# grunwaldlab/krisp

Measured on AMD Instinct MI355X. Metric: k-mers/s sorted+intersected at k=28, higher is better.
Workload: dtype u64

## Files before the change

### include/krisp_hip.h

```cpp
#ifndef KRISP_HIP_H
#define KRISP_HIP_H

#include <stddef.h>
#include <stdint.h>

#ifdef __cplusplus
extern "C" {
#endif

typedef struct kr_ctx kr_ctx;

typedef struct { uint64_t prefix, in_mask, out_mask; } kr_cand;

typedef struct { uint64_t key; uint32_t genome; uint32_t count; } kr_record;

enum {
    KR_OK = 0,
    KR_ERR_HIP = -1,
    KR_ERR_PARAM = -2,
    KR_ERR_CAPACITY = -3,
    KR_ERR_STATE = -4,
    KR_ERR_KEY = -5,
    KR_ERR_HOST = -6
};
// ... 193 lines not shown
       KR_OPT_COARSE_POOL = 12,
       KR_OPT_JOIN2 = 13,
       KR_OPT_WIDE_ORDERED = 6 };
int     kr_set_option(kr_ctx*, int option, int64_t value);

int     kr_sync(kr_ctx*);
int     kr_timer_begin(kr_ctx*);
double  kr_timer_end_ms(kr_ctx*);
int     kr_stage_enable(kr_ctx*, int on);
int     kr_stage_select(kr_ctx*, unsigned stage_mask);
int     kr_stage_reset(kr_ctx*);
double  kr_stage_ms(kr_ctx*, int stage);
int64_t kr_stage_launches(kr_ctx*, int stage);

int64_t kr_debug_fetch(kr_ctx*, int genome_id, int what, void* out, size_t cap_bytes);
int64_t kr_debug_inversions(kr_ctx*, int genome_id);
double  kr_debug_localsort(kr_ctx*, int genome_id, int reps, int mode);
double  kr_debug_intersect(kr_ctx*, const int* genome_ids, int n, const uint8_t* is_ingroup, int reps, int mode);
double  kr_debug_copy_gbps(kr_ctx*, size_t bytes, int reps);
const char* kr_debug_copy_which(kr_ctx*);
int     kr_build_experiments(void);
int     kr_debug_lazy(kr_ctx*, int64_t* out8);
int     kr_debug_isect(kr_ctx*, int64_t* out8);
int     kr_debug_scan(kr_ctx*, int64_t* out8);
int     kr_debug_place(kr_ctx*, double* out8);
int     kr_debug_coarse_pool(kr_ctx*, double* out8);
int     kr_debug_comm(kr_ctx*, int64_t* out8);
int     kr_debug_comm_probe(kr_ctx*, size_t bytes, int reps, double* out3);
int64_t kr_debug_cands_selfexchange(kr_ctx*, int apply_filter);
int     kr_debug_comm_hang(kr_ctx*);
int64_t kr_debug_budget_left(kr_ctx*);
int     kr_debug_budget_set(kr_ctx*, int64_t left);
int     kr_debug_info(kr_ctx*, int64_t* out8);

#ifdef __cplusplus
}
#endif
#endif
```

### krisp_amd/_native.py

```python
import ctypes
import os

import numpy as np

HERE = os.path.dirname(os.path.abspath(__file__))
LIB_PATH = os.environ.get("KRISP_HIP_LIB") or os.path.join(HERE, "libkrisp_hip.so")

CAND = np.dtype([("prefix", "<u8"), ("in_mask", "<u8"), ("out_mask", "<u8")])
RECORD = np.dtype([("key", "<u8"), ("genome", "<u4"), ("count", "<u4")])
WIDE_HIT = np.dtype([("cand", "<u4"), ("genome", "<u4"), ("pos", "<u4"), ("strand", "<u4")])
LOC_HIT = np.dtype([("group", "<u4"), ("strand", "<u4"), ("pos", "<u8")])
NEAR_HIT = np.dtype([("target", "<u4"), ("strand", "u1"), ("mismatches", "u1"), ("flank_mismatches", "u1"), ("pad", "u1"),
                     ("pos", "<u8")])
PRODUCT_SITE = np.dtype([("pos", "<u8"), ("entry", "<u4"), ("mismatches", "u1"), ("end_mismatches", "u1"),
                         ("pad", "<u2")])
PRODUCT_HIT = np.dtype([("pos", "<u8"), ("length", "<u4"), ("pair", "<u4"), ("strand", "u1"), ("left_mm", "u1"),
                        ("right_mm", "u1"), ("left_end_mm", "u1"), ("right_end_mm", "u1"), ("pad", "u1", (3,))])
DESIGN_RECORD = np.dtype([("found", "<u4"), ("product_size", "<u4"), ("pair_penalty", "<u4"), ("left_start", "<u2"),
                          ("left_len", "<u2"), ("right_start", "<u2"), ("right_len", "<u2"), ("left_tm", "<i4"), ("right_tm", "<i4"),
                          ("left_gc", "<u2"), ("right_gc", "<u2"), ("left_penalty", "<u4"), ("right_penalty", "<u4"),
                          ("left_self_any", "<i4"), ("left_self_end", "<i4"), ("right_self_any", "<i4"),
                          ("right_self_end", "<i4"), ("pair_any", "<i4"), ("pair_end", "<i4")])
DESIGN_RECORD_HP = np.dtype(DESIGN_RECORD.descr + [("left_hairpin", "<i4"), ("right_hairpin", "<i4")])
GUIDE_RECORD = np.dtype([("found", "<u4"), ("strand", "<u4"), ("start", "<u4"), ("min_mismatches", "<u4"),
# ... 125 lines not shown
    ("kr_timer_end_ms", _c.c_double, [_P]),
    ("kr_stage_enable", _c.c_int, [_P, _c.c_int]),
    ("kr_stage_select", _c.c_int, [_P, _c.c_uint]),
    ("kr_stage_reset", _c.c_int, [_P]),
    ("kr_stage_ms", _c.c_double, [_P, _c.c_int]),
    ("kr_stage_launches", _c.c_int64, [_P, _c.c_int]),
    ("kr_debug_fetch", _c.c_int64, [_P, _c.c_int, _c.c_int, _P, _c.c_size_t]),
    ("kr_debug_inversions", _c.c_int64, [_P, _c.c_int]),
    ("kr_debug_localsort", _c.c_double, [_P, _c.c_int, _c.c_int, _c.c_int]),
    ("kr_debug_intersect", _c.c_double, [_P, _P, _c.c_int, _P, _c.c_int, _c.c_int]),
    ("kr_debug_copy_gbps", _c.c_double, [_P, _c.c_size_t, _c.c_int]),
    ("kr_debug_copy_which", _c.c_char_p, [_P]),
    ("kr_mem_info", _c.c_int, [_P, _P]),
    ("kr_debug_comm", _c.c_int, [_P, _P]),
    ("kr_debug_place", _c.c_int, [_P, _P]),
    ("kr_debug_coarse_pool", _c.c_int, [_P, _P]),
    ("kr_debug_comm_probe", _c.c_int, [_P, _c.c_size_t, _c.c_int, _P]),
    ("kr_debug_cands_selfexchange", _c.c_int64, [_P, _c.c_int]),
    ("kr_debug_info", _c.c_int, [_P, _P]),
    ("kr_render_records", _c.c_int64, [_P, _c.c_size_t, _c.c_int, _c.c_int, _c.c_int, _P, _c.c_size_t, _P, _c.c_size_t, _P,
                                       _c.c_int, _P, _P, _P, _P]),
    ("kr_text_free", None, [_P]),
    ("kr_debug_isect", _c.c_int, [_P, _P]),
    ("kr_debug_lazy", _c.c_int, [_P, _P]),
    ("kr_debug_scan", _c.c_int, [_P, _P]),
    ("kr_set_mixed_alphabets", _c.c_int, [_P, _c.c_int]),
    ("kr_build_experiments", _c.c_int, []),
    ("kr_comm_set_timeout", _c.c_int, [_P, _c.c_int]),
    ("kr_debug_comm_hang", _c.c_int, [_P]),
    ("kr_debug_budget_left", _c.c_int64, [_P]),
    ("kr_debug_budget_set", _c.c_int, [_P, _c.c_int64]),
]


class GuideParams(ctypes.Structure):
    _fields_ = [("guide_size", _c.c_int32), ("pam5_len", _c.c_int32), ("pam3_len", _c.c_int32), ("pam5", _c.c_uint8 * 8),
                ("pam3", _c.c_uint8 * 8), ("gc_lo", _c.c_int32), ("gc_hi", _c.c_int32), ("min_mismatches", _c.c_int32)]


class KrispHipError(RuntimeError):
    code = None


ERR_CAPACITY = -3


# ... 629 lines not shown
        for n in names:
            mask |= 1 << STAGES.index(n)
        self.lib.kr_stage_select(self.ctx, mask)

    def stage_reset(self):
        self.lib.kr_stage_reset(self.ctx)

    def stage_times(self):
        return {name: (self.lib.kr_stage_ms(self.ctx, i), self.lib.kr_stage_launches(self.ctx, i))
                for i, name in enumerate(STAGES)}

    def debug_info(self):
        o = np.zeros(8, dtype=np.int64)
        self.lib.kr_debug_info(self.ctx, _ptr(o))
        return dict(b=int(o[0]), nbuckets=int(o[1]), T=int(o[2]), CAP=int(o[3]), nwg=int(o[4]),
                    overflow_segments=int(o[5]), fallback_launches=int(o[6]), nslices=int(o[7]))

    def debug_isect(self):
        o = np.zeros(8, dtype=np.int64)
        self.lib.kr_debug_isect(self.ctx, _ptr(o))
        return dict(chunk_kernel_items=int(o[0]), slices_redone=int(o[1]), threads=int(o[2]), buckets_per_item_log2=int(o[3]),
                    heads32=int(o[4]), sort_lanes=int(o[5]), join2_launches=int(o[6]), join2_handed_on=int(o[7]))

    def debug_lazy(self):
        o = np.zeros(8, dtype=np.int64)
        self.lib.kr_debug_lazy(self.ctx, _ptr(o))
        return dict(skipped=int(o[0]), ordered_later=int(o[1]), touch_collects=int(o[2]), on=int(o[3]),
                    anchor_in_bucket_order=int(o[4]), fuse_anchor=int(o[5]), coarse=int(o[6]), coarse_promoted=int(o[7]))

    def debug_scan(self):
        o = np.zeros(8, dtype=np.int64)
        self.lib.kr_debug_scan(self.ctx, _ptr(o))
        return dict(tiles=int(o[0]), grid=int(o[1]), cap=int(o[2]), blocks=int(o[3]))

    def copy_gbps(self, nbytes=1 << 30, reps=10):
        v = self.lib.kr_debug_copy_gbps(self.ctx, nbytes, reps)
        if v < 0:
            raise KrispHipError("kr_debug_copy_gbps failed")
        return v

    def mem_info(self):
        o = np.zeros(4, dtype=np.int64)
        self._check(self.lib.kr_mem_info(self.ctx, _ptr(o)), "kr_mem_info")
        return dict(avail=int(o[0]), total=int(o[1]), used=int(o[2]), budget=int(o[3]))

    def debug_comm(self):
# ... 44 lines not shown
```

### krisp_amd/csrc/h_core.inc

```
static thread_local std::string g_last_error;

struct DevBuf {
    void* p = nullptr;
    size_t bytes = 0;
};

struct Slice {
    DevBuf keys, off, chunkstart, chunkdesc, ovf;
    u64 nmax = 0;
    u32 nchunks = 0;
    int64_t count = -1;
    int res = -1;
};

struct Genome {
    int id = -1;
    size_t n_bases = 0;
    u64 nwords = 0;
    u64 nmax = 0;
    DevBuf bases, wkeys;
    DevBuf wlcnt;
    bool wlist = false;
    u32 wlcap = 0;
    std::vector<Slice> sl;
// ... 63 lines not shown
    bool stage_on = false;
    unsigned stage_mask = ~0u;
    struct Pair { hipEvent_t a, b; int stage; };
    std::vector<Pair> pending;
    std::vector<hipEvent_t> pool;
    double stage_ms[KR_ST_COUNT] = {0};
    int64_t stage_n[KR_ST_COUNT] = {0};
    int64_t fallback_launches = 0, overflow_segments = 0;
    int dbg = 0;
    int isect_kernel = 0;
    int ncu = 256;
    DevBuf bgz_in, bgz_tab, bgz_stat;
    DevBuf tx_scan;
    DevBuf tx_text, tx_tile, tx_tilepos, tx_lines, tx_ls, tx_ll, tx_op, tx_outpos, tx_state, tx_tsum, tx_tpos;
    u32* mbox = nullptr;
    std::vector<uint64_t> coltab_host;
    std::vector<int> mb_free;
    int mb_next = 0;
    int i3_occ[3][4][9] = {{{0}}};
    DevBuf isovf;
    int join2 = 1;
    u32 j2_grid = 0;
    int j2_occ[9] = {0};
    int64_t j2_launches = 0, j2_full = 0;
    bool j2_full_counted = false;
    int64_t isect_ovf_items = 0, isect_refall = 0;
    int i3_last_T = 0, i3_last_mlog = 0, i3_last_tags = 0, i3_last_ua = 0;
    int64_t isect_ua = 0;
    int fuse_anchor = 1;
    u32 i3_ovf_cap = I3_OVF_CAP;
    int isect_fmt = 0;
    int opt_slice_bases = -1;
    hipEvent_t slice_ready[2] = {nullptr, nullptr};
    bool custom_layout = false;
    bool mixed_alphabets = false;
    int lazy_order = 1;
    bool order_wanted = false;
    int64_t lazy_skipped = 0, lazy_ordered = 0, lazy_touch = 0;
    DevBuf touchdesc, touchovf;
    int coarse_rest = 1;
    int64_t coarse_done = 0, coarse_promoted = 0;
    int coarse_pool = 1;
    struct PoolBuf { DevBuf buf; double ms; hipEvent_t ev; bool wait; };
    std::vector<PoolBuf> cpool_free;
    int cpool_total = 0;
    int64_t cpool_partitions = 0;
// ... 457 lines not shown
    }
    c->stream = c->lanes[0].stream;
    return c;
}

int kr_comm_destroy(kr_ctx* c);

void kr_destroy(kr_ctx* c) {
    if (!c) return;
    (void)kr_comm_destroy(c);
    (void)hipSetDevice(c->device);
    (void)hipDeviceSynchronize();
    resolve_stages(c);
    for (int i = 0; i < MAX_LANES; i++) {
        Lane& ln = c->lanes[i];
        DevBuf* lb[] = {&ln.codes, &ln.bad, &ln.partial8, &ln.base1, &ln.tmpkeys, &ln.tp, &ln.tiledesc, &ln.tilehist, &ln.wkeys,
                        &ln.pass0, &ln.base64, &ln.partial16, &ln.cursor, &ln.h16exc, &ln.slt, &ln.offa, &ln.cura};
        for (DevBuf* b : lb) release(c, *b);
    }
    for (auto& kv : c->genomes) release_genome(c, kv.second);
    coarse_pool_release(c);
    DevBuf* all[] = {&c->candA, &c->candB, &c->chunkcnt,
                     &c->chunkpos, &c->flags, &c->blockcnt, &c->blockpos, &c->other, &c->records, &c->nrec, &c->fbdesc, &c->fbsegs,
                     &c->coltab, &c->collo, &c->colcnt, &c->colpos, &c->coltsum, &c->coltpos, &c->colfirst, &c->colfm, &c->isovf,
                     &c->bgz_in, &c->bgz_tab, &c->bgz_stat, &c->tx_scan, &c->tx_text, &c->tx_tile, &c->tx_tilepos, &c->tx_lines, &c->tx_ls, &c->tx_ll, &c->tx_op, &c->tx_outpos, &c->tx_state,
                     &c->tx_tsum, &c->tx_tpos, &c->candP, &c->touchdesc, &c->touchovf, &c->co_state, &c->co_tab};
    for (DevBuf* b : all) release(c, *b);
    {
        auto& w = c->wide;
        DevBuf* wb[] = {&w.fin.keys, &w.fin.idx, &w.fin.slots, &w.masks, &w.keep, &w.cnt, &w.hitoff, &w.cursor, &w.hits,
                        &w.cibuf, &w.loc, &w.loccur, &w.tsum, &w.tpos, &w.wcount, &w.flbuf, &w.rows, &w.rowtab};
        for (DevBuf* b : wb) release(c, *b);
        for (int f = 0; f < 2; f++)
            for (int q = 0; q < 2 * FR_MAXP - 1; q++) {
                auto& d = w.fd[f][q];
                release(c, d.keys); release(c, d.idx); release(c, d.slots); release(c, d.mzT); release(c, d.mzB);
            }
    }
    {
        kr_ctx::Bufs sb;
        c->loc.bufs(sb); c->near.bufs(sb); c->ghit.bufs(sb); c->gbulge.bufs(sb); c->prod.bufs(sb); c->prim.bufs(sb);
        for (DevBuf* b : sb) release(c, *b);
        auto& ds = c->design;
        DevBuf* db[] = {&ds.par, &ds.tmpl, &ds.rec, &ds.hprec};
        for (DevBuf* b : db) release(c, *b);
        auto& gu = c->guides;
        DevBuf* gb[] = {&gu.rows, &gu.off, &gu.bnd, &gu.rec};
// ... 1274 lines not shown
```

### krisp_amd/csrc/h_intersect.inc

```
static int64_t intersect_once(kr_ctx* c, const int* ids, int n, const uint8_t* is_in, int apply_filter, bool* redo);

static int64_t cands_merge_device(kr_ctx* c, size_t m, int have_other, int apply_filter);

static inline int fmode(const kr_ctx* c, int apply_filter) { return apply_filter ? (c->mixed_alphabets ? 2 : 1) : 0; }

int kr_set_mixed_alphabets(kr_ctx* c, int on) {
    if (!c) return KR_ERR_PARAM;
    c->mixed_alphabets = on != 0;
    return KR_OK;
}

#define KR_MAX_CANDS 0xFFFFFF00ull
static int cands_fit(kr_ctx* c, uint64_t n, const char* who) {
    if (n < KR_MAX_CANDS) return KR_OK;
    return fail(c, KR_ERR_CAPACITY, "%s: a candidate list of %llu entries exceeds the %llu a list may hold (an intersection that "
                "nothing prunes: give both ingroup and outgroup genomes to one call, or fewer genomes per call)", who,
                (unsigned long long)n, (unsigned long long)KR_MAX_CANDS);
}

static int cands_compact_room(kr_ctx* c, u32 n) {
    const size_t nblk = ((size_t)n + 255) / 256;
    int rc;
    if ((rc = ensure(c, c->flags, (size_t)n * 4))) return rc;
    if ((rc = ensure(c, c->blockcnt, (nblk + 2) * 4))) return rc;
// ... 299 lines not shown
            const int mlog = ip.mlog;
            const u32 T = ip.T;
            const bool tagk = ip.tagk;
            const bool ua = tagk && !gs[anchor]->ordered;
            a3.n = n;
            a3.ingroup_bits = ingroup_bits;
            a3.anchor = anchor;
            a3.apply_filter = a.apply_filter;
            for (int i = 0; i < n; i++) { a3.keys[i] = a.keys[i]; a3.off[i] = a.off[i]; }
            a3.nb = nbk;
            a3.mlog = mlog;
            a3.nitems = (nbk + (1u << mlog) - 1) >> mlog;
            a3.sh = tagk ? ip.sht : std::max(g.rb + mlog - (int)I3_NB_LOG, ip.p0);
            a3.p0 = ip.p0;
            a3.tmp = (kr_cand*)c->candA.p;
            a3.itemcnt = (u32*)c->chunkcnt.p;
            a3.ovf = (u32*)c->isovf.p;
            a3.ovf_cap = c->i3_ovf_cap;
            c->i3_last_T = (int)T;
            c->i3_last_mlog = mlog;
            nunits = a3.nitems;
            c->i3_last_tags = tagk ? 1 : 0;
            const bool st32 = tagk && fmt == 0 && g.D == 1 && n <= 24 && c->isect_fmt == 0;
            const bool join2 = c->join2 && n == 2 && (ingroup_bits == 1u || ingroup_bits == 2u) && a.apply_filter == 1 &&
                               g.D == 1 && tagk && ip.p0 >= 2 && c->isect_fmt == 0 && c->isect_kernel == 0 && c->fuse_anchor != 0;
            const Isect3Kernel kern = join2 ? k_join2 : isect3_kernel(ua, tagk, st32, fmt);
            int& occ = join2 ? c->j2_occ[T / 64] : c->i3_occ[ua ? 2 : (tagk ? 1 : 0)][st32 ? 3 : fmt][T / 64];
            if (occ == 0) {
                int per = 0;
                const hipError_t e = hipOccupancyMaxActiveBlocksPerMultiprocessor(&per, kern, (int)T, 0);
                occ = (e == hipSuccess && per >= 1) ? per : 1;
            }
            u32 grid = std::min<u32>(a3.nitems, (u32)(occ * c->ncu));
            if (join2 && c->j2_grid) grid = std::min(grid, c->j2_grid);
            {
                StageScope sc(c, KR_ST_INTERSECT, st);
                c->i3_last_ua = ua ? 1 : 0;
                if (ua) c->isect_ua++;
                if (join2) c->j2_launches++;
                hipLaunchKernelGGL(kern, dim3(grid), dim3(T), 0, st, a3, g);
                a.ovf = (const u32*)c->isovf.p;
                a.ovf_cap = c->i3_ovf_cap;
                a.mlog = mlog;
                a.nb = nbk;
                if (all_ordered) launch_chunks(I3_OVF_LAUNCH);
            }
        } else {
            StageScope sc(c, KR_ST_INTERSECT, st);
            launch_chunks(AS.nchunks);
        }
        u32 total = 0;
        auto gather = [&](u32 cap) {
            if (by_items)
                hipLaunchKernelGGL(k_gather_items, dim3((nunits + GI_ITEMS - 1) / GI_ITEMS), dim3(GI_T), 0, st, g.sbits, g.slice,
                                   (const kr_cand*)c->candA.p, (const u32*)AS.off.p, a3.mlog, nbk,
                                   (const u32*)c->chunkcnt.p, (const u32*)c->chunkpos.p, (kr_cand*)c->candB.p + running,
                                   nunits, cap);
            else
                hipLaunchKernelGGL(k_gather_cands, dim3(AS.nchunks), dim3(64), 0, st, g.sbits, g.slice,
                                   (const kr_cand*)c->candA.p, (const uint4*)AS.chunkdesc.p,
                                   (const u32*)c->chunkcnt.p, (const u32*)c->chunkpos.p,
                                   (kr_cand*)c->candB.p + running, nunits, cap);
        };
// ... 387 lines not shown
```

### krisp_amd/csrc/h_misc.inc

```
double kr_debug_localsort(kr_ctx* c, int id, int reps, int mode) {
    if (!c || mode != 0) return -1.0;
    auto it = c->genomes.find(id);
    if (it != c->genomes.end() && ensure_fine(c, it->second)) return -1.0;
    if (it == c->genomes.end() || !it->second.sorted || it->second.sl.empty()) return -1.0;
    if (ensure_ordered(c, {&it->second}) || finalize(c, {&it->second})) return -1.0;
    Slice& S = it->second.sl[0];
    hipStream_t st = c->stream;
    const u32 grid = std::min<u32>(S.nchunks, (u32)c->ls_grid);
    auto launch = [&]() {
        hipLaunchKernelGGL(k_localsort2, dim3(grid), dim3(LS_THREADS), 0, st, (u64*)S.keys.p, (const u32*)S.off.p,
                           (const uint4*)S.chunkdesc.p, S.nchunks, c->g.b, (u32*)S.ovf.p,
                           (uint4*)((char*)S.ovf.p + 16));
    };
    hipEvent_t a, b;
    (void)hipEventCreate(&a);
    (void)hipEventCreate(&b);
    launch();
    (void)hipEventRecord(a, st);
    for (int r = 0; r < reps; r++) launch();
    (void)hipEventRecord(b, st);
    (void)hipEventSynchronize(b);
    float ms = 0;
    (void)hipEventElapsedTime(&ms, a, b);
    (void)hipEventDestroy(a);
// ... 237 lines not shown
    out8[1] = (double)c->cpool_free.size();
    out8[2] = held;
    out8[3] = (double)c->cpool_partitions;
    out8[4] = (double)c->cpool_searches;
    out8[5] = lo;
    out8[6] = hi;
    out8[7] = c->coarse_pool;
    return KR_OK;
}

int kr_debug_isect(kr_ctx* c, int64_t* o) {
    if (!c || !o) return KR_ERR_PARAM;
    o[0] = c->isect_ovf_items;
    o[1] = c->isect_refall;
    o[2] = c->i3_last_T;
    o[3] = c->i3_last_mlog;
    o[4] = c->i3_last_tags;
    o[5] = lanes_used(c);
    o[6] = c->j2_launches;
    o[7] = c->j2_full;
    return KR_OK;
}

int kr_debug_scan(kr_ctx* c, int64_t* o) {
    if (!c || !o) return KR_ERR_PARAM;
    o[0] = c->scan_dbg[0];
    o[1] = c->scan_dbg[1];
    o[2] = c->scan_cap;
    o[3] = c->scan_dbg[2];
    o[4] = o[5] = o[6] = o[7] = 0;
    return KR_OK;
}

int kr_build_experiments(void) {
    int bits = 0;
#ifdef KR_EXPERIMENTS
    bits |= 1;
#endif
#ifdef KR_ABLATE
    bits |= 2;
#endif
#if defined(I3_ABL) && I3_ABL
    bits |= 4;
#endif
#if defined(P2_ABL) && P2_ABL
    bits |= 8;
// ... 39 lines not shown
```

### krisp_amd/csrc/k_join2.inc

```
#include "j2_screen.inc"

#ifndef J2_OCC
#define J2_OCC 6
#endif
#define J2_FULL_WORD (I3_OVF_CAP + 2)

__global__ __launch_bounds__(I3_MAXT, J2_OCC) void k_join2(Isect3Args a, Geom g) {
    __shared__ __attribute__((aligned(16))) u32 scr[J2_SCREEN / 4];
    __shared__ __attribute__((aligned(16))) unsigned long long tkey[J2_TAB];
    __shared__ __attribute__((aligned(16))) u32 tst[J2_TAB];
    __shared__ unsigned long long lkey[J2_TAB];
    __shared__ u32 lst[J2_TAB];
    __shared__ uint2 rng[2][MAXG];
    __shared__ const u64* keyp[MAXG];
    __shared__ u32 ctl[2];
    const u32 tid = threadIdx.x, T = blockDim.x, S = 4 * T, G = gridDim.x;
    const u32 lane = tid & 63;
    const bool anchor_in = (a.ingroup_bits >> a.anchor) & 1;
    const int p0 = a.p0, wbits = a.sh + (int)I3T_NB_LOG - a.p0;
    const u32 prA = 1u << (8 + a.anchor), prB = 1u << (8 + (1 - a.anchor));
    const u32 sdA = anchor_in ? 1u : 16u, sdB = anchor_in ? 16u : 1u;
    const u32 og = min(lane >> 1, (u32)a.n - 1);
    const u32 __attribute__((address_space(1)))* myoff;
    {
        u64 mo = (u64)a.off[og];
        asm volatile("" : "+v"(mo));
        myoff = (const u32 __attribute__((address_space(1)))*)mo;
    }
    auto item_bucket = [&](u32 it, u32 which) {
        const u64 f = ((u64)it + which) << a.mlog;
        return (u32)(f < a.nb ? f : a.nb);
    };
    for (u32 i = tid; i < J2_SCREEN / 4; i += T) scr[i] = 0;
    for (u32 i = tid; i < J2_TAB; i += T) { tkey[i] = 0; tst[i] = 0; }
    if (tid < 2) ctl[tid] = 0;
    if (tid < (u32)a.n) keyp[tid] = a.keys[tid];
    {
        u32 v = myoff[item_bucket(blockIdx.x, lane & 1)];
        asm volatile("" : "+v"(v));
        if (tid < 2 * (u32)a.n) {
            if (lane & 1) rng[0][og].y = v; else rng[0][og].x = v;
        }
    }
    __syncthreads();
    I3State cur;
    cur.it = blockIdx.x;
    cur.g = -1;
    cur.par = 0;
    {
        const uint2 r = rng[0][a.anchor];
        const u32 s = i3_uni(r.x), e = i3_uni(r.y);
        cur.over = (e - s > S) ? 1u : 0u;
        cur.i0 = s;
        cur.e = cur.over ? s : e;
    }
    if (cur.it >= a.nitems) return;
    u32 item_sa = 0, item_cnt = 0;
    u32 item_full = 0, item_firstb = 0;
    u32 voff = 0;
    I3Regs X, Y, KA;
    KA.q[0] = KA.q[1] = u32x4{0, 0, 0, 0};
    i3_issue(X, a, keyp, cur, T);

    auto ikey_of = [&](u32 lo, u32 hi) { return j2_item_key(((u64)hi << 32) | lo, p0, wbits); };
    auto base_of = [&](u32 lo) { return __builtin_amdgcn_ubfe(lo, (u32)(p0 - 2), 2u); };
    auto insert = [&](u64 ik, u32 sw) {
        const unsigned long long want = ik | (1ull << 63);
        u32 h = j2_tab_hash(ik);
        bool placed = false;
        for (u32 t = 0; t < J2_PROBES && !placed; t++) {
            const unsigned long long old = atomicCAS(&tkey[h], 0ull, want);
            if (old == 0ull || old == want) {
                atomicOr(&tst[h], sw);
                placed = true;
            }
            h = (h + 1) & (J2_TAB - 1);
        }
        if (!placed) ctl[1] = 1;
    };
    auto probe = [&](u64 ik, u32 sw) {
        const unsigned long long want = ik | (1ull << 63);
        u32 h = j2_tab_hash(ik);
        for (u32 t = 0; t < J2_PROBES; t++) {
            const unsigned long long old = tkey[h];
            if (old == want) atomicOr(&tst[h], sw);
            if (old == want || old == 0ull) break;
            h = (h + 1) & (J2_TAB - 1);
        }
    };
    auto list_item = [&](u32 it, bool full) {
        const u32 idx = atomicAdd(&a.ovf[0], 1u);
        if (idx < a.ovf_cap) a.ovf[1 + idx] = it;
        if (full) atomicAdd(&a.ovf[J2_FULL_WORD], 1u);
        a.itemcnt[it] = 0;
    };

    auto advance = [&](I3State& st, u32& pass, u32& b0) {
        if (st.g >= 0 && st.i0 + S < st.e) {
            st.i0 += S;
        } else if (st.g < 0) {
            const uint2 r = rng[st.par][1 - a.anchor];
            st.g = 1 - a.anchor;
            st.i0 = i3_uni(r.x);
            st.e = st.over ? st.i0 : i3_uni(r.y);
            b0 = st.i0;
            pass = 0;
        } else if (pass == 0 && st.e - b0 > S) {
            st.i0 = b0;
            pass = 1;
        } else {
            st.it += G;
            st.par ^= 1u;
            st.g = -1;
            pass = 0;
            const uint2 r = rng[st.par][a.anchor];
            const u32 s = i3_uni(r.x), e = i3_uni(r.y);
            st.over = (e - s > S) ? 1u : 0u;
            st.i0 = s;
            st.e = st.over ? s : e;
        }
        if (st.it >= a.nitems) { st.i0 = 0; st.e = 0; st.over = 0; }
        st.it = i3_uni(st.it); st.g = (int)i3_uni((u32)st.g); st.i0 = i3_uni(st.i0); st.e = i3_uni(st.e);
        st.par = i3_uni(st.par); st.over = i3_uni(st.over);
        pass = i3_uni(pass); b0 = i3_uni(b0);
    };

    auto process = [&](const I3Regs& R, const I3State& st, const u32 pass, const I3State& nx) {
        const u32 tid = opaque_tid();
        asm volatile("" ::"v"(R.q[0]), "v"(R.q[1]));
        if (st.g < 0) {
            item_sa = st.i0;
            item_cnt = st.e - st.i0;
            item_full = 0;
            item_firstb = 1;
            const u32 cnt = item_cnt;
            if (st.over) {
                if (tid == 0) list_item(st.it, false);
            } else {
#pragma unroll
                for (int e = 0; e < 4; e++)
                    if (I3_POS(e) < cnt) {
                        const u32 slot = j2_slot(ikey_of(I3_LO(R, e), I3_HI(R, e)));
                        atomicOr(&scr[slot >> 2], j2_bit(slot, base_of(I3_LO(R, e)), false));
                    }
                KA = R;
            }
            if (tid < 2 * (u32)a.n) {
                if (lane & 1) rng[st.par ^ 1u][og].y = voff; else rng[st.par ^ 1u][og].x = voff;
            }
            __syncthreads();
        } else if (!st.over) {
            const u32 cnt = item_cnt;
            const u32 left = st.e - st.i0;
            const bool last_of_pass = !(st.i0 + S < st.e);
            if (item_firstb) {
                if (tid == 0) ctl[0] = 0;
                item_firstb = 0;
            }
            if (pass == 0) {
#pragma unroll
                for (int e = 0; e < 4; e++)
                    if (I3_POS(e) < left) {
                        const u32 slot = j2_slot(ikey_of(I3_LO(R, e), I3_HI(R, e)));
                        atomicOr(&scr[slot >> 2], j2_bit(slot, base_of(I3_LO(R, e)), true));
                    }
                if (last_of_pass) {
                    __syncthreads();
#pragma unroll
                    for (int e = 0; e < 4; e++)
                        if (I3_POS(e) < cnt) {
                            const u64 ik = ikey_of(I3_LO(KA, e), I3_HI(KA, e));
                            const u32 slot = j2_slot(ik);
                            if (j2_live_byte(j2_byte(scr[slot >> 2], slot))) insert(ik, prA | (sdA << base_of(I3_LO(KA, e))));
                        }
                    __syncthreads();
                    item_full = i3_uni(ctl[1]);
                }
            }
            if ((nx.it != st.it || pass == 1) && !item_full) {
#pragma unroll
                for (int e = 0; e < 4; e++)
                    if (I3_POS(e) < left) {
                        const u64 ik = ikey_of(I3_LO(R, e), I3_HI(R, e));
                        const u32 slot = j2_slot(ik);
                        if (j2_live_byte(j2_byte(scr[slot >> 2], slot))) probe(ik, prB | (sdB << base_of(I3_LO(R, e))));
                    }
            }
            if (nx.it != st.it) {
                __syncthreads();
                const bool full = item_full != 0;
                for (u32 i = tid; i < J2_TAB; i += T) {
                    const unsigned long long k = tkey[i];
                    if (k != 0ull) {
                        const u32 s = tst[i];
                        tkey[i] = 0ull;
                        tst[i] = 0;
                        if (!full && (s >> 8) == 3u && (s & (s >> 4) & 15u) == 0) {
                            const u32 idx = atomicAdd(&ctl[0], 1u);
                            lkey[idx] = k;
                            lst[idx] = s;
                        }
                    }
                }
                for (u32 i = 4 * tid; i < J2_SCREEN / 4; i += 4 * T) *reinterpret_cast<uint4*>(&scr[i]) = make_uint4(0, 0, 0, 0);
                if (tid == 0) ctl[1] = 0;
                __syncthreads();
                const u32 nsurv = full ? 0u : i3_uni(ctl[0]);
                if (nsurv) {
                    const u64 base = ((u64)st.it << a.mlog) << g.rb;
                    const u64 wmask = (1ull << wbits) - 1;
                    kr_cand* out = a.tmp + item_sa;
                    for (u32 i = tid; i < nsurv; i += T) {
                        const unsigned long long k = lkey[i];
                        const u32 s = lst[i];
                        u32 r = 0;
                        for (u32 j = 0; j < nsurv; j++) r += lkey[j] < k ? 1u : 0u;
                        kr_cand c;
                        c.prefix = base | ((k & wmask) << p0);
                        c.in_mask = (u64)(s & 15u);
                        c.out_mask = (u64)((s >> 4) & 15u);
                        out[r] = c;
                    }
                }
                if (tid == 0) {
                    if (full) list_item(st.it, true);
                    else a.itemcnt[st.it] = nsurv;
                }
            }
        }
    };

    u32 cur_pass = 0, b0 = 0;
    for (;;) {
        I3State nxt = cur;
        u32 nxt_pass = cur_pass;
        if (cur.g < 0) {
            const u32 ni = cur.it + G < a.nitems ? cur.it + G : 0u;
            voff = myoff[item_bucket(ni, lane & 1)];
        }
        advance(nxt, nxt_pass, b0);
        i3_issue(Y, a, keyp, nxt, T);
        process(X, cur, cur_pass, nxt);
        cur = nxt;
        cur_pass = nxt_pass;
        if (cur.it >= a.nitems) break;
        if (cur.g < 0) {
            const u32 ni = cur.it + G < a.nitems ? cur.it + G : 0u;
            voff = myoff[item_bucket(ni, lane & 1)];
        }
        advance(nxt, nxt_pass, b0);
        i3_issue(X, a, keyp, nxt, T);
        process(Y, cur, cur_pass, nxt);
        cur = nxt;
        cur_pass = nxt_pass;
        if (cur.it >= a.nitems) break;
    }
}
```

Measured before the change: 128.1 billion.

## Split join2 into screen-and-append kernel plus single-wave hash-join kernel

The fused join2 kernel is split in two. The first kernel screens both genomes' keys through a double-buffered LDS bitmap and appends only the surviving keys to global per-item lists, recording per-item live counts. The second kernel is a one-wave workgroup that prefetches those short lists, builds and probes the LDS hash table, and ranks and writes the candidates. The aim is to drop the large hash tables from the screening kernel so it can run at higher occupancy (J2_OCC raised from 6 to 7), and to let the join run many small waves in parallel. The cost is an extra launch, extra global traffic for the live lists, and new scratch buffers.

```diff
diff --git a/include/krisp_hip.h b/include/krisp_hip.h
--- a/include/krisp_hip.h
+++ b/include/krisp_hip.h
@@ -239,6 +239,7 @@
 int     kr_build_experiments(void);
 int     kr_debug_lazy(kr_ctx*, int64_t* out8);
 int     kr_debug_isect(kr_ctx*, int64_t* out8);
+int     kr_debug_join2(kr_ctx*, int64_t* out8);
 int     kr_debug_scan(kr_ctx*, int64_t* out8);
 int     kr_debug_place(kr_ctx*, double* out8);
 int     kr_debug_coarse_pool(kr_ctx*, double* out8);
diff --git a/krisp_amd/_native.py b/krisp_amd/_native.py
--- a/krisp_amd/_native.py
+++ b/krisp_amd/_native.py
@@ -171,6 +171,7 @@
                                        _c.c_int, _P, _P, _P, _P]),
     ("kr_text_free", None, [_P]),
     ("kr_debug_isect", _c.c_int, [_P, _P]),
+    ("kr_debug_join2", _c.c_int, [_P, _P]),
     ("kr_debug_lazy", _c.c_int, [_P, _P]),
     ("kr_debug_scan", _c.c_int, [_P, _P]),
     ("kr_set_mixed_alphabets", _c.c_int, [_P, _c.c_int]),
@@ -846,6 +847,13 @@
         return dict(chunk_kernel_items=int(o[0]), slices_redone=int(o[1]), threads=int(o[2]), buckets_per_item_log2=int(o[3]),
                     heads32=int(o[4]), sort_lanes=int(o[5]), join2_launches=int(o[6]), join2_handed_on=int(o[7]))
 
+    def debug_join2(self):
+        o = np.zeros(8, dtype=np.int64)
+        rc = self.lib.kr_debug_join2(self.ctx, _ptr(o))
+        if rc < 0:
+            raise KrispHipError("kr_debug_join2 failed")
+        return dict(live_anchor=int(o[0]), live_other=int(o[1]), live_items=int(o[2]), marked_items=int(o[3]), items=int(o[4]))
+
     def debug_lazy(self):
         o = np.zeros(8, dtype=np.int64)
         self.lib.kr_debug_lazy(self.ctx, _ptr(o))
diff --git a/krisp_amd/csrc/h_core.inc b/krisp_amd/csrc/h_core.inc
--- a/krisp_amd/csrc/h_core.inc
+++ b/krisp_amd/csrc/h_core.inc
@@ -109,6 +109,9 @@
     int join2 = 1;
     u32 j2_grid = 0;
     int j2_occ[9] = {0};
+    int j2l_occ = 0;
+    DevBuf j2_blive, j2_la, j2_lb;
+    u32 j2_last_items = 0;
     int64_t j2_launches = 0, j2_full = 0;
     bool j2_full_counted = false;
     int64_t isect_ovf_items = 0, isect_refall = 0;
@@ -612,7 +615,7 @@
     coarse_pool_release(c);
     DevBuf* all[] = {&c->candA, &c->candB, &c->chunkcnt,
                      &c->chunkpos, &c->flags, &c->blockcnt, &c->blockpos, &c->other, &c->records, &c->nrec, &c->fbdesc, &c->fbsegs,
-                     &c->coltab, &c->collo, &c->colcnt, &c->colpos, &c->coltsum, &c->coltpos, &c->colfirst, &c->colfm, &c->isovf,
+                     &c->coltab, &c->collo, &c->colcnt, &c->colpos, &c->coltsum, &c->coltpos, &c->colfirst, &c->colfm, &c->isovf, &c->j2_blive, &c->j2_la, &c->j2_lb,
                      &c->bgz_in, &c->bgz_tab, &c->bgz_stat, &c->tx_scan, &c->tx_text, &c->tx_tile, &c->tx_tilepos, &c->tx_lines, &c->tx_ls, &c->tx_ll, &c->tx_op, &c->tx_outpos, &c->tx_state,
                      &c->tx_tsum, &c->tx_tpos, &c->candP, &c->touchdesc, &c->touchovf, &c->co_state, &c->co_tab};
     for (DevBuf* b : all) release(c, *b);
diff --git a/krisp_amd/csrc/h_intersect.inc b/krisp_amd/csrc/h_intersect.inc
--- a/krisp_amd/csrc/h_intersect.inc
+++ b/krisp_amd/csrc/h_intersect.inc
@@ -345,14 +345,34 @@
             nunits = a3.nitems;
             c->i3_last_tags = tagk ? 1 : 0;
             const bool st32 = tagk && fmt == 0 && g.D == 1 && n <= 24 && c->isect_fmt == 0;
-            const bool join2 = c->join2 && n == 2 && (ingroup_bits == 1u || ingroup_bits == 2u) && a.apply_filter == 1 &&
-                               g.D == 1 && tagk && ip.p0 >= 2 && c->isect_fmt == 0 && c->isect_kernel == 0 && c->fuse_anchor != 0;
-            const Isect3Kernel kern = join2 ? k_join2 : isect3_kernel(ua, tagk, st32, fmt);
+            bool join2 = c->join2 && n == 2 && (ingroup_bits == 1u || ingroup_bits == 2u) && a.apply_filter == 1 &&
+                         g.D == 1 && tagk && ip.p0 >= 2 && c->isect_fmt == 0 && c->isect_kernel == 0 && c->fuse_anchor != 0;
+            J2Lists jl{};
+            if (join2) {
+                const std::string err0 = c->err;
+                if (ensure(c, c->j2_blive, ((size_t)gs[1 - anchor]->sl[s].nmax + 2) * 8) ||
+                    ensure(c, c->j2_la, ((size_t)a3.nitems + 2) * 4) || ensure(c, c->j2_lb, ((size_t)a3.nitems + 2) * 4)) {
+                    join2 = false;
+                    c->err = err0;
+                    g_last_error = err0;
+                }
+                jl.blive = (u64*)c->j2_blive.p;
+                jl.la = (u32*)c->j2_la.p;
+                jl.lb = (u32*)c->j2_lb.p;
+            }
+            c->j2_last_items = join2 ? a3.nitems : 0u;
+            const Isect3Kernel kern = isect3_kernel(ua, tagk, st32, fmt);
             int& occ = join2 ? c->j2_occ[T / 64] : c->i3_occ[ua ? 2 : (tagk ? 1 : 0)][st32 ? 3 : fmt][T / 64];
             if (occ == 0) {
                 int per = 0;
-                const hipError_t e = hipOccupancyMaxActiveBlocksPerMultiprocessor(&per, kern, (int)T, 0);
+                const hipError_t e = join2 ? hipOccupancyMaxActiveBlocksPerMultiprocessor(&per, k_join2, (int)T, 0)
+                                           : hipOccupancyMaxActiveBlocksPerMultiprocessor(&per, kern, (int)T, 0);
                 occ = (e == hipSuccess && per >= 1) ? per : 1;
+            }
+            if (join2 && c->j2l_occ == 0) {
+                int per = 0;
+                const hipError_t e = hipOccupancyMaxActiveBlocksPerMultiprocessor(&per, k_join2_live, J2L_T, 0);
+                c->j2l_occ = (e == hipSuccess && per >= 1) ? per : 1;
             }
             u32 grid = std::min<u32>(a3.nitems, (u32)(occ * c->ncu));
             if (join2 && c->j2_grid) grid = std::min(grid, c->j2_grid);
@@ -360,8 +380,15 @@
                 StageScope sc(c, KR_ST_INTERSECT, st);
                 c->i3_last_ua = ua ? 1 : 0;
                 if (ua) c->isect_ua++;
-                if (join2) c->j2_launches++;
-                hipLaunchKernelGGL(kern, dim3(grid), dim3(T), 0, st, a3, g);
+                if (join2) {
+                    u32 grid2 = std::min<u32>(a3.nitems, (u32)(c->j2l_occ * c->ncu));
+                    if (c->j2_grid) grid2 = std::min(grid2, c->j2_grid);
+                    c->j2_launches++;
+                    hipLaunchKernelGGL(k_join2, dim3(grid), dim3(T), 0, st, a3, g, jl);
+                    hipLaunchKernelGGL(k_join2_live, dim3(grid2), dim3(J2L_T), 0, st, a3, g, jl);
+                } else {
+                    hipLaunchKernelGGL(kern, dim3(grid), dim3(T), 0, st, a3, g);
+                }
                 a.ovf = (const u32*)c->isovf.p;
                 a.ovf_cap = c->i3_ovf_cap;
                 a.mlog = mlog;
diff --git a/krisp_amd/csrc/h_misc.inc b/krisp_amd/csrc/h_misc.inc
--- a/krisp_amd/csrc/h_misc.inc
+++ b/krisp_amd/csrc/h_misc.inc
@@ -283,6 +283,26 @@
     return KR_OK;
 }
 
+int kr_debug_join2(kr_ctx* c, int64_t* o) {
+    if (!c || !o) return KR_ERR_PARAM;
+    for (int i = 0; i < 8; i++) o[i] = 0;
+    const u32 ni = c->j2_last_items;
+    if (ni == 0 || !c->j2_la.p || !c->j2_lb.p) return KR_OK;
+    HIPCHK(c, hipSetDevice(c->device));
+    HIPCHK(c, hipStreamSynchronize(c->stream));
+    std::vector<u32> la(ni), lb(ni);
+    HIPCHK(c, hipMemcpy(la.data(), c->j2_la.p, (size_t)ni * 4, hipMemcpyDeviceToHost));
+    HIPCHK(c, hipMemcpy(lb.data(), c->j2_lb.p, (size_t)ni * 4, hipMemcpyDeviceToHost));
+    for (u32 i = 0; i < ni; i++) {
+        if (la[i] == J2_LIVE_SKIP) { o[3]++; continue; }
+        o[0] += la[i];
+        o[1] += lb[i];
+        o[2] += (la[i] | lb[i]) != 0;
+    }
+    o[4] = ni;
+    return KR_OK;
+}
+
 int kr_debug_scan(kr_ctx* c, int64_t* o) {
     if (!c || !o) return KR_ERR_PARAM;
     o[0] = c->scan_dbg[0];
diff --git a/krisp_amd/csrc/j2_live.inc b/krisp_amd/csrc/j2_live.inc
--- /dev/null
+++ b/krisp_amd/csrc/j2_live.inc
@@ -0,0 +1,18 @@
+#include <stdint.h>
+
+#define J2_LIVE_SKIP 0xFFFFFFFFu
+
+__host__ __device__ inline uint32_t j2_item_bucket(uint32_t it, uint32_t which, int mlog, uint32_t nb) {
+    const uint64_t f = ((uint64_t)it + which) << mlog;
+    return (uint32_t)(f < nb ? f : nb);
+}
+
+__host__ __device__ inline uint64_t j2_alive_word(uint32_t sa, uint32_t cnt, uint32_t pos) { return 3ull * sa + cnt + pos; }
+__host__ __device__ inline bool j2_alive_ok(uint32_t cnt, uint32_t pos) { return pos < cnt; }
+
+__host__ __device__ inline uint64_t j2_blive_word(uint32_t sb, uint32_t pos) { return (uint64_t)sb + pos; }
+__host__ __device__ inline bool j2_blive_ok(uint32_t bn, uint32_t pos) { return pos < bn; }
+
+__host__ __device__ inline bool j2_counts_ok(uint32_t la, uint32_t lb, uint32_t cnt, uint32_t bn) {
+    return la != J2_LIVE_SKIP && la <= cnt && lb <= bn;
+}
diff --git a/krisp_amd/csrc/k_join2.inc b/krisp_amd/csrc/k_join2.inc
--- a/krisp_amd/csrc/k_join2.inc
+++ b/krisp_amd/csrc/k_join2.inc
@@ -1,25 +1,38 @@
 #include "j2_screen.inc"
+#include "j2_live.inc"
 
 #ifndef J2_OCC
-#define J2_OCC 6
+#define J2_OCC 7
+#endif
+#ifndef J2L_T
+#define J2L_T 64
+#endif
+#ifndef J2L_PRE
+#define J2L_PRE 3
 #endif
 #define J2_FULL_WORD (I3_OVF_CAP + 2)
 
-__global__ __launch_bounds__(I3_MAXT, J2_OCC) void k_join2(Isect3Args a, Geom g) {
-    __shared__ __attribute__((aligned(16))) u32 scr[J2_SCREEN / 4];
-    __shared__ __attribute__((aligned(16))) unsigned long long tkey[J2_TAB];
-    __shared__ __attribute__((aligned(16))) u32 tst[J2_TAB];
-    __shared__ unsigned long long lkey[J2_TAB];
-    __shared__ u32 lst[J2_TAB];
+struct J2Lists {
+    u64* blive;
+    u32* la;
+    u32* lb;
+};
+
+__device__ __forceinline__ void j2_list_item(const Isect3Args& a, u32 it, bool full) {
+    const u32 idx = atomicAdd(&a.ovf[0], 1u);
+    if (idx < a.ovf_cap) a.ovf[1 + idx] = it;
+    if (full) atomicAdd(&a.ovf[J2_FULL_WORD], 1u);
+    a.itemcnt[it] = 0;
+}
+
+__global__ __launch_bounds__(I3_MAXT, J2_OCC) void k_join2(Isect3Args a, Geom g, J2Lists l) {
+    __shared__ __attribute__((aligned(16))) u32 scr[2][J2_SCREEN / 4];
     __shared__ uint2 rng[2][MAXG];
     __shared__ const u64* keyp[MAXG];
-    __shared__ u32 ctl[2];
+    __shared__ u32 lcnt[2][2];
     const u32 tid = threadIdx.x, T = blockDim.x, S = 4 * T, G = gridDim.x;
     const u32 lane = tid & 63;
-    const bool anchor_in = (a.ingroup_bits >> a.anchor) & 1;
     const int p0 = a.p0, wbits = a.sh + (int)I3T_NB_LOG - a.p0;
-    const u32 prA = 1u << (8 + a.anchor), prB = 1u << (8 + (1 - a.anchor));
-    const u32 sdA = anchor_in ? 1u : 16u, sdB = anchor_in ? 16u : 1u;
     const u32 og = min(lane >> 1, (u32)a.n - 1);
     const u32 __attribute__((address_space(1)))* myoff;
     {
@@ -27,16 +40,11 @@
         asm volatile("" : "+v"(mo));
         myoff = (const u32 __attribute__((address_space(1)))*)mo;
     }
-    auto item_bucket = [&](u32 it, u32 which) {
-        const u64 f = ((u64)it + which) << a.mlog;
-        return (u32)(f < a.nb ? f : a.nb);
-    };
-    for (u32 i = tid; i < J2_SCREEN / 4; i += T) scr[i] = 0;
-    for (u32 i = tid; i < J2_TAB; i += T) { tkey[i] = 0; tst[i] = 0; }
-    if (tid < 2) ctl[tid] = 0;
+    for (u32 i = tid; i < 2 * (J2_SCREEN / 4); i += T) (&scr[0][0])[i] = 0;
+    if (tid < 4) lcnt[tid >> 1][tid & 1] = 0;
     if (tid < (u32)a.n) keyp[tid] = a.keys[tid];
     {
-        u32 v = myoff[item_bucket(blockIdx.x, lane & 1)];
+        u32 v = myoff[j2_item_bucket(blockIdx.x, lane & 1, a.mlog, a.nb)];
         asm volatile("" : "+v"(v));
         if (tid < 2 * (u32)a.n) {
             if (lane & 1) rng[0][og].y = v; else rng[0][og].x = v;
@@ -56,7 +64,9 @@
     }
     if (cur.it >= a.nitems) return;
     u32 item_sa = 0, item_cnt = 0;
-    u32 item_full = 0, item_firstb = 0;
+    u32 item_sb = 0, item_bn = 0;
+    u32 item_firstb = 0;
+    u32 prev_it = 0, prev_par = 0, have_prev = 0;
     u32 voff = 0;
     I3Regs X, Y, KA;
     KA.q[0] = KA.q[1] = u32x4{0, 0, 0, 0};
@@ -64,35 +74,36 @@
 
     auto ikey_of = [&](u32 lo, u32 hi) { return j2_item_key(((u64)hi << 32) | lo, p0, wbits); };
     auto base_of = [&](u32 lo) { return __builtin_amdgcn_ubfe(lo, (u32)(p0 - 2), 2u); };
-    auto insert = [&](u64 ik, u32 sw) {
-        const unsigned long long want = ik | (1ull << 63);
-        u32 h = j2_tab_hash(ik);
-        bool placed = false;
-        for (u32 t = 0; t < J2_PROBES && !placed; t++) {
-            const unsigned long long old = atomicCAS(&tkey[h], 0ull, want);
-            if (old == 0ull || old == want) {
-                atomicOr(&tst[h], sw);
-                placed = true;
-            }
-            h = (h + 1) & (J2_TAB - 1);
-        }
-        if (!placed) ctl[1] = 1;
-    };
-    auto probe = [&](u64 ik, u32 sw) {
-        const unsigned long long want = ik | (1ull << 63);
-        u32 h = j2_tab_hash(ik);
-        for (u32 t = 0; t < J2_PROBES; t++) {
-            const unsigned long long old = tkey[h];
-            if (old == want) atomicOr(&tst[h], sw);
-            if (old == want || old == 0ull) break;
-            h = (h + 1) & (J2_TAB - 1);
-        }
-    };
-    auto list_item = [&](u32 it, bool full) {
-        const u32 idx = atomicAdd(&a.ovf[0], 1u);
-        if (idx < a.ovf_cap) a.ovf[1 + idx] = it;
-        if (full) atomicAdd(&a.ovf[J2_FULL_WORD], 1u);
-        a.itemcnt[it] = 0;
+    auto flush = [&](u32 it, u32 par) {
+        l.la[it] = lcnt[par][0];
+        l.lb[it] = lcnt[par][1];
+        lcnt[par][0] = 0;
+        lcnt[par][1] = 0;
+    };
+    auto append = [&](const I3Regs& R, const u32* sc, u32 lim, u32 par, u32 which, u64* dst, u32 room) {
+        const u32 tid = opaque_tid();
+        bool lv[4];
+        u32 below[4], n[4];
+#pragma unroll
+        for (int e = 0; e < 4; e++) {
+            const u32 slot = j2_slot(ikey_of(I3_LO(R, e), I3_HI(R, e)));
+            lv[e] = I3_POS(e) < lim && j2_live_byte(j2_byte(sc[slot >> 2], slot));
+            const unsigned long long m = __ballot(lv[e]);
+            below[e] = __builtin_amdgcn_mbcnt_hi((u32)(m >> 32), __builtin_amdgcn_mbcnt_lo((u32)m, 0u));
+            n[e] = (u32)__popcll(m);
+        }
+        const u32 tot = n[0] + n[1] + n[2] + n[3];
+        if (tot) {
+            u32 at = 0;
+            if (lane == 0) at = atomicAdd(&lcnt[par][which], tot);
+            at = i3_uni(at);
+#pragma unroll
+            for (int e = 0; e < 4; e++) {
+                const u32 pos = at + below[e];
+                if (lv[e] && (which ? j2_blive_ok(room, pos) : j2_alive_ok(room, pos))) dst[pos] = ((u64)I3_HI(R, e) << 32) | I3_LO(R, e);
+                at += n[e];
+            }
+        }
     };
 
     auto advance = [&](I3State& st, u32& pass, u32& b0) {
@@ -128,20 +139,18 @@
     auto process = [&](const I3Regs& R, const I3State& st, const u32 pass, const I3State& nx) {
         const u32 tid = opaque_tid();
         asm volatile("" ::"v"(R.q[0]), "v"(R.q[1]));
+        u32* const sc = scr[st.par];
         if (st.g < 0) {
             item_sa = st.i0;
             item_cnt = st.e - st.i0;
-            item_full = 0;
             item_firstb = 1;
             const u32 cnt = item_cnt;
-            if (st.over) {
-                if (tid == 0) list_item(st.it, false);
-            } else {
+            if (!st.over) {
 #pragma unroll
                 for (int e = 0; e < 4; e++)
                     if (I3_POS(e) < cnt) {
                         const u32 slot = j2_slot(ikey_of(I3_LO(R, e), I3_HI(R, e)));
-                        atomicOr(&scr[slot >> 2], j2_bit(slot, base_of(I3_LO(R, e)), false));
+                        atomicOr(&sc[slot >> 2], j2_bit(slot, base_of(I3_LO(R, e)), false));
                     }
                 KA = R;
             }
@@ -149,12 +158,28 @@
                 if (lane & 1) rng[st.par ^ 1u][og].y = voff; else rng[st.par ^ 1u][og].x = voff;
             }
             __syncthreads();
+            if (tid == 0) {
+                if (have_prev) flush(prev_it, prev_par);
+                if (st.over) {
+                    j2_list_item(a, st.it, false);
+                    l.la[st.it] = J2_LIVE_SKIP;
+                    l.lb[st.it] = 0;
+                }
+            }
+            {
+                u32* const old = scr[st.par ^ 1u];
+                for (u32 i = 4 * tid; i < J2_SCREEN / 4; i += 4 * T) *reinterpret_cast<uint4*>(&old[i]) = make_uint4(0, 0, 0, 0);
+            }
+            have_prev = st.over ? 0u : 1u;
+            prev_it = st.it;
+            prev_par = st.par;
+            if (st.over) __syncthreads();
         } else if (!st.over) {
-            const u32 cnt = item_cnt;
             const u32 left = st.e - st.i0;
             const bool last_of_pass = !(st.i0 + S < st.e);
             if (item_firstb) {
-                if (tid == 0) ctl[0] = 0;
+                item_sb = st.i0;
+                item_bn = st.e - st.i0;
                 item_firstb = 0;
             }
             if (pass == 0) {
@@ -162,71 +187,15 @@
                 for (int e = 0; e < 4; e++)
                     if (I3_POS(e) < left) {
                         const u32 slot = j2_slot(ikey_of(I3_LO(R, e), I3_HI(R, e)));
-                        atomicOr(&scr[slot >> 2], j2_bit(slot, base_of(I3_LO(R, e)), true));
+                        atomicOr(&sc[slot >> 2], j2_bit(slot, base_of(I3_LO(R, e)), true));
                     }
                 if (last_of_pass) {
                     __syncthreads();
-#pragma unroll
-                    for (int e = 0; e < 4; e++)
-                        if (I3_POS(e) < cnt) {
-                            const u64 ik = ikey_of(I3_LO(KA, e), I3_HI(KA, e));
-                            const u32 slot = j2_slot(ik);
-                            if (j2_live_byte(j2_byte(scr[slot >> 2], slot))) insert(ik, prA | (sdA << base_of(I3_LO(KA, e))));
-                        }
-                    __syncthreads();
-                    item_full = i3_uni(ctl[1]);
+                    append(KA, sc, item_cnt, st.par, 0u, (u64*)a.tmp + j2_alive_word(item_sa, item_cnt, 0u), item_cnt);
                 }
             }
-            if ((nx.it != st.it || pass == 1) && !item_full) {
-#pragma unroll
-                for (int e = 0; e < 4; e++)
-                    if (I3_POS(e) < left) {
-                        const u64 ik = ikey_of(I3_LO(R, e), I3_HI(R, e));
-                        const u32 slot = j2_slot(ik);
-                        if (j2_live_byte(j2_byte(scr[slot >> 2], slot))) probe(ik, prB | (sdB << base_of(I3_LO(R, e))));
-                    }
-            }
-            if (nx.it != st.it) {
-                __syncthreads();
-                const bool full = item_full != 0;
-                for (u32 i = tid; i < J2_TAB; i += T) {
-                    const unsigned long long k = tkey[i];
-                    if (k != 0ull) {
-                        const u32 s = tst[i];
-                        tkey[i] = 0ull;
-                        tst[i] = 0;
-                        if (!full && (s >> 8) == 3u && (s & (s >> 4) & 15u) == 0) {
-                            const u32 idx = atomicAdd(&ctl[0], 1u);
-                            lkey[idx] = k;
-                            lst[idx] = s;
-                        }
-                    }
-                }
-                for (u32 i = 4 * tid; i < J2_SCREEN / 4; i += 4 * T) *reinterpret_cast<uint4*>(&scr[i]) = make_uint4(0, 0, 0, 0);
-                if (tid == 0) ctl[1] = 0;
-                __syncthreads();
-                const u32 nsurv = full ? 0u : i3_uni(ctl[0]);
-                if (nsurv) {
-                    const u64 base = ((u64)st.it << a.mlog) << g.rb;
-                    const u64 wmask = (1ull << wbits) - 1;
-                    kr_cand* out = a.tmp + item_sa;
-                    for (u32 i = tid; i < nsurv; i += T) {
-                        const unsigned long long k = lkey[i];
-                        const u32 s = lst[i];
-                        u32 r = 0;
-                        for (u32 j = 0; j < nsurv; j++) r += lkey[j] < k ? 1u : 0u;
-                        kr_cand c;
-                        c.prefix = base | ((k & wmask) << p0);
-                        c.in_mask = (u64)(s & 15u);
-                        c.out_mask = (u64)((s >> 4) & 15u);
-                        out[r] = c;
-                    }
-                }
-                if (tid == 0) {
-                    if (full) list_item(st.it, true);
-                    else a.itemcnt[st.it] = nsurv;
-                }
-            }
+            if (nx.it != st.it || pass == 1)
+                append(R, sc, left, st.par, 1u, l.blive + j2_blive_word(item_sb, 0u), item_bn);
         }
     };
 
@@ -236,7 +205,7 @@
         u32 nxt_pass = cur_pass;
         if (cur.g < 0) {
             const u32 ni = cur.it + G < a.nitems ? cur.it + G : 0u;
-            voff = myoff[item_bucket(ni, lane & 1)];
+            voff = myoff[j2_item_bucket(ni, lane & 1, a.mlog, a.nb)];
         }
         advance(nxt, nxt_pass, b0);
         i3_issue(Y, a, keyp, nxt, T);
@@ -246,7 +215,7 @@
         if (cur.it >= a.nitems) break;
         if (cur.g < 0) {
             const u32 ni = cur.it + G < a.nitems ? cur.it + G : 0u;
-            voff = myoff[item_bucket(ni, lane & 1)];
+            voff = myoff[j2_item_bucket(ni, lane & 1, a.mlog, a.nb)];
         }
         advance(nxt, nxt_pass, b0);
         i3_issue(X, a, keyp, nxt, T);
@@ -255,4 +224,195 @@
         cur_pass = nxt_pass;
         if (cur.it >= a.nitems) break;
     }
+    __syncthreads();
+    if (tid == 0 && have_prev) flush(prev_it, prev_par);
 }
+
+__device__ __forceinline__ void j2_wave_sync() {
+    __builtin_amdgcn_fence(__ATOMIC_RELEASE, "wavefront");
+    __builtin_amdgcn_wave_barrier();
+    __builtin_amdgcn_fence(__ATOMIC_ACQUIRE, "wavefront");
+}
+struct J2Meta { u32 la, lb, sa, cnt, sb, bn; };
+static_assert(J2L_T == 64, "k_join2_live: a workgroup is one wave");
+
+__global__ __launch_bounds__(J2L_T) void k_join2_live(Isect3Args a, Geom g, J2Lists l) {
+    __shared__ __attribute__((aligned(16))) unsigned long long tkey[J2_TAB + 8];
+    __shared__ __attribute__((aligned(16))) u32 tst[J2_TAB];
+    __shared__ u32 turns[6][J2L_T];
+    const u32 tid = threadIdx.x, G = gridDim.x;
+    const bool anchor_in = (a.ingroup_bits >> a.anchor) & 1;
+    const int p0 = a.p0, wbits = a.sh + (int)I3T_NB_LOG - a.p0;
+    const u32 prA = 1u << (8 + a.anchor), prB = 1u << (8 + (1 - a.anchor));
+    const u32 sdA = anchor_in ? 1u : 16u, sdB = anchor_in ? 16u : 1u;
+    const u32* offA = a.off[a.anchor];
+    const u32* offB = a.off[1 - a.anchor];
+    for (u32 i = tid; i < J2_TAB + 8; i += J2L_T) tkey[i] = 0;
+    for (u32 i = tid; i < J2_TAB; i += J2L_T) tst[i] = 0;
+    j2_wave_sync();
+    auto load_turns = [&](u32 t0) {
+        const u32 it = blockIdx.x + (t0 + tid) * G;
+        J2Meta m{J2_LIVE_SKIP, 0, 0, 0, 0, 0};
+        if (it < a.nitems) {
+            const u32 bk0 = j2_item_bucket(it, 0, a.mlog, a.nb), bk1 = j2_item_bucket(it, 1, a.mlog, a.nb);
+            m.la = l.la[it];
+            m.lb = l.lb[it];
+            m.sa = offA[bk0];
+            m.cnt = offA[bk1] - m.sa;
+            m.sb = offB[bk0];
+            m.bn = offB[bk1] - m.sb;
+        }
+        j2_wave_sync();
+        turns[0][tid] = m.la; turns[1][tid] = m.lb; turns[2][tid] = m.sa;
+        turns[3][tid] = m.cnt; turns[4][tid] = m.sb; turns[5][tid] = m.bn;
+        j2_wave_sync();
+    };
+    auto turn_meta = [&](u32 t) {
+        if ((t & 63u) == 0) load_turns(t);
+        J2Meta m;
+        m.la = i3_uni(turns[0][t & 63u]); m.lb = i3_uni(turns[1][t & 63u]); m.sa = i3_uni(turns[2][t & 63u]);
+        m.cnt = i3_uni(turns[3][t & 63u]); m.sb = i3_uni(turns[4][t & 63u]); m.bn = i3_uni(turns[5][t & 63u]);
+        return m;
+    };
+    auto joins = [&](const J2Meta& m) { return m.la != 0 && m.lb != 0 && j2_counts_ok(m.la, m.lb, m.cnt, m.bn); };
+    auto alist = [&](const J2Meta& m) { return (const u64*)a.tmp + j2_alive_word(m.sa, m.cnt, 0u); };
+    auto blist = [&](const J2Meta& m) { return (const u64*)l.blive + j2_blive_word(m.sb, 0u); };
+    auto fetch = [&](const J2Meta& m, u64* ka, u64* kb) {
+#pragma unroll
+        for (u32 r = 0; r < J2L_PRE; r++) ka[r] = kb[r] = 0;
+        if (joins(m)) {
+#pragma unroll
+            for (u32 r = 0; r < J2L_PRE; r++) {
+                if (tid + r * J2L_T < m.la) ka[r] = alist(m)[tid + r * J2L_T];
+                if (tid + r * J2L_T < m.lb) kb[r] = blist(m)[tid + r * J2L_T];
+            }
+        }
+    };
+    auto insert = [&](u64 key) {
+        const u64 ik = j2_item_key(key, p0, wbits);
+        const u32 sw = prA | (sdA << __builtin_amdgcn_ubfe((u32)key, (u32)(p0 - 2), 2u));
+        const unsigned long long want = ik | (1ull << 63);
+        u32 h = j2_tab_hash(ik);
+        bool placed = false;
+        for (u32 t = 0; t < J2_PROBES && !placed; t++) {
+            const unsigned long long old = atomicCAS(&tkey[h], 0ull, want);
+            if (old == 0ull || old == want) {
+                atomicOr(&tst[h], sw);
+                placed = true;
+            }
+            h = (h + 1) & (J2_TAB - 1);
+        }
+        return placed;
+    };
+    auto probe = [&](u64 key) {
+        const u64 ik = j2_item_key(key, p0, wbits);
+        const u32 sw = prB | (sdB << __builtin_amdgcn_ubfe((u32)key, (u32)(p0 - 2), 2u));
+        const unsigned long long want = ik | (1ull << 63);
+        u32 h = j2_tab_hash(ik);
+        for (u32 t = 0; t < J2_PROBES; t++) {
+            const unsigned long long old = tkey[h];
+            if (old == want) atomicOr(&tst[h], sw);
+            if (old == want || old == 0ull) break;
+            h = (h + 1) & (J2_TAB - 1);
+        }
+    };
+
+    auto join_item = [&](const J2Meta& m, const u64* ka0, const u64* kb0, u32 it) {
+        if (m.la != J2_LIVE_SKIP && !joins(m)) {
+            if (tid == 0) a.itemcnt[it] = 0;
+        } else if (m.la != J2_LIVE_SKIP) {
+            const u32 la = m.la, lb = m.lb, cnt = m.cnt;
+            bool nofit = false;
+#pragma unroll
+            for (u32 r = 0; r < J2L_PRE; r++)
+                if (tid + r * J2L_T < la) nofit = !insert(ka0[r]) || nofit;
+            for (u32 i = tid + J2L_PRE * J2L_T; i < la; i += J2L_T) nofit = !insert(alist(m)[i]) || nofit;
+            const bool full = __any(nofit) != 0;
+            j2_wave_sync();
+            if (!full) {
+#pragma unroll
+                for (u32 r = 0; r < J2L_PRE; r++)
+                    if (tid + r * J2L_T < lb) probe(kb0[r]);
+                for (u32 i = tid + J2L_PRE * J2L_T; i < lb; i += J2L_T) probe(blist(m)[i]);
+            }
+            j2_wave_sync();
+            constexpr u32 PER = J2_TAB / J2L_T;
+            unsigned long long k[PER];
+            u32 st[PER], pos[PER];
+            u32 nsurv = 0;
+#pragma unroll
+            for (u32 e = 0; e < PER; e++) {
+                k[e] = tkey[tid + e * J2L_T];
+                st[e] = tst[tid + e * J2L_T];
+            }
+#pragma unroll
+            for (u32 e = 0; e < PER; e++) {
+                if (k[e] != 0ull) {
+                    tkey[tid + e * J2L_T] = 0ull;
+                    tst[tid + e * J2L_T] = 0;
+                }
+                const bool keep = !full && k[e] != 0ull && (st[e] >> 8) == 3u && (st[e] & (st[e] >> 4) & 15u) == 0;
+                const unsigned long long mk = __ballot(keep);
+                pos[e] = keep ? nsurv + __builtin_amdgcn_mbcnt_hi((u32)(mk >> 32), __builtin_amdgcn_mbcnt_lo((u32)mk, 0u)) : ~0u;
+                nsurv += (u32)__popcll(mk);
+            }
+            j2_wave_sync();
+            if (nsurv) {
+#pragma unroll
+                for (u32 e = 0; e < PER; e++)
+                    if (pos[e] != ~0u) {
+                        tkey[pos[e]] = k[e];
+                        tst[pos[e]] = st[e];
+                    }
+                j2_wave_sync();
+                const u64 base = ((u64)it << a.mlog) << g.rb;
+                const u64 wmask = (1ull << wbits) - 1;
+                kr_cand* out = a.tmp + m.sa;
+                for (u32 i = tid; i < nsurv; i += J2L_T) {
+                    const unsigned long long ki = tkey[i];
+                    const u32 s = tst[i];
+                    u32 r = 0;
+                    for (u32 j = 0; j < nsurv; j += 8) {
+                        unsigned long long o[8];
+#pragma unroll
+                        for (u32 u = 0; u < 8; u++) o[u] = tkey[j + u];
+#pragma unroll
+                        for (u32 u = 0; u < 8; u++) r += (j + u < nsurv && o[u] < ki) ? 1u : 0u;
+                    }
+                    kr_cand c;
+                    c.prefix = base | ((ki & wmask) << p0);
+                    c.in_mask = (u64)(s & 15u);
+                    c.out_mask = (u64)((s >> 4) & 15u);
+                    if (r < cnt) out[r] = c;
+                }
+                j2_wave_sync();
+                for (u32 i = tid; i < nsurv; i += J2L_T) {
+                    tkey[i] = 0ull;
+                    tst[i] = 0;
+                }
+                j2_wave_sync();
+            }
+            if (tid == 0) {
+                if (full) j2_list_item(a, it, true);
+                else a.itemcnt[it] = nsurv;
+            }
+        }
+    };
+
+    u64 pa[J2L_PRE], pb[J2L_PRE], qa[J2L_PRE], qb[J2L_PRE];
+    u32 t = 0;
+    J2Meta mp = turn_meta(0), mq;
+    fetch(mp, pa, pb);
+    for (u32 it = blockIdx.x;;) {
+        mq = turn_meta(++t);
+        fetch(mq, qa, qb);
+        join_item(mp, pa, pb, it);
+        it += G;
+        if (it >= a.nitems) break;
+        mp = turn_meta(++t);
+        fetch(mp, pa, pb);
+        join_item(mq, qa, qb, it);
+        it += G;
+        if (it >= a.nitems) break;
+    }
+}
```

Measured after the change: 125.7 billion. 1.9% lower.
